# MarkJhonBao/InfantPoseEstimation_GaussianBias

Hardware: AMD Instinct MI355X
Metric: images/sec (train fwd+bwd) HRFormer-S 256x192 (higher is better)
Workload: dtype bf16; 1 GPU; HRFormer-small + fusion head, 256x192 -> 64x48, K=17, train step fwd+bwd+AdamW, DropPath 0.1, BN train; global_batch=64, per_gpu_batch=64, parallelism=dp1, launch=hipGraph replay, branches on concurrent HIP streams

## Files before the change

infantposeestimation_gaussianbias_amd/csrc/pk_layout.hip:

```cpp
#include "pk_rowops.h"

__global__ void __launch_bounds__(256) k_nchw_to_nhwc(const float* __restrict__ x, uint16_t* __restrict__ y, int B, int Cin, int H, int W,
                                                      int Cp, const float* __restrict__ sp_y) {
    const size_t pixels = (size_t)B * H * W;
    for (size_t i = (size_t)blockIdx.x * blockDim.x + threadIdx.x; i < pixels; i += (size_t)gridDim.x * blockDim.x) {
        const size_t b = i / ((size_t)H * W), r = i - b * H * W;
        for (int c0 = 0; c0 < Cp; c0 += 8) {
            float v[8];
#pragma unroll
            for (int j = 0; j < 8; ++j) {
                float t = 0.f;
                if (c0 + j < Cin) {
                    const size_t k = (b * Cin + c0 + j) * H * W + r;
                    t = x[k];
                    if (sp_y) t *= 1.f - __expf(-sp_y[k]);
                }
                v[j] = t;
            }
            *reinterpret_cast<uint4*>(y + i * Cp + c0) = pack8(v);
        }
    }
}
extern "C" int pk_nchw_f32_to_nhwc_bf16(const float* x, const float* softplus_out, void* y, int B, int Cin, int H, int W, int Cpad,
                                        void* stream) {
    PK_REQUIRE(x && y && B > 0 && Cin > 0 && H > 0 && W > 0 && Cpad >= Cin && (Cpad & 7) == 0, "pk_nchw_f32_to_nhwc_bf16: bad argument");
    const size_t pixels = (size_t)B * H * W;
    unsigned gb;
    chunk_grid(pixels, 1, CHUNK_GRID_CAP, nullptr, gb);
    hipLaunchKernelGGL(k_nchw_to_nhwc, dim3(gb), dim3(256), 0, (hipStream_t)stream, x, (uint16_t*)y, B, Cin, H, W, Cpad, softplus_out);
    return pk_launch_status("pk_nchw_f32_to_nhwc_bf16");
}

struct PackDesc { const float* src; int64_t dst_off; int N, C, T, mode, Cp, Np; int64_t dst_numel; };
__global__ void __launch_bounds__(256) k_pack_weights(uint16_t* __restrict__ dst, const PackDesc* __restrict__ desc,
                                                      const int* __restrict__ blk_desc, const int* __restrict__ blk_first) {
    const PackDesc d = desc[blk_desc[blockIdx.x]];
    const float* __restrict__ src = d.src;
    const int64_t i0 = (int64_t)(blockIdx.x - blk_first[blockIdx.x]) * 1024;
    for (int k = 0; k < 4; ++k) {
        const int64_t i = i0 + k * 256 + threadIdx.x;
        if (i >= d.dst_numel) return;
        float v = 0.f;
        if (d.mode == 0) {
            const int c = (int)(i % d.Cp), t = (int)((i / d.Cp) % d.T), n = (int)(i / ((int64_t)d.Cp * d.T));
            if (c < d.C) v = src[((int64_t)n * d.C + c) * d.T + t];
        } else if (d.mode == 1) {
            const int n = (int)(i % d.Np), t = (int)((i / d.Np) % d.T), c = (int)(i / ((int64_t)d.Np * d.T));
            if (n < d.N) v = src[((int64_t)n * d.C + c) * d.T + (d.T - 1 - t)];
        } else {
            const int n = (int)(i % d.Np), c = (int)(i / d.Np);
            if (n < d.N) v = src[(int64_t)n * d.C + c];
        }
        dst[d.dst_off + i] = f32_to_bf16(v);
    }
}
extern "C" int pk_pack_weights(void* flat_dst_bf16, const void* desc_table, const int32_t* block_desc, const int32_t* block_first,
                               int n_blocks, void* stream) {
    PK_REQUIRE(flat_dst_bf16 && desc_table && block_desc && block_first && n_blocks > 0, "pk_pack_weights: bad argument");
    hipLaunchKernelGGL(k_pack_weights, dim3(n_blocks), dim3(256), 0, (hipStream_t)stream, (uint16_t*)flat_dst_bf16,
                       (const PackDesc*)desc_table, block_desc, block_first);
    return pk_launch_status("pk_pack_weights");
}

struct EmbedDesc { float* real; int64_t twin_off; int r[4]; int p[4]; int64_t numel; };
__global__ void __launch_bounds__(256) k_embed_boxes(float* __restrict__ twin, const EmbedDesc* __restrict__ desc,
                                                     const int* __restrict__ blk_desc, const int* __restrict__ blk_first, int direction) {
    const EmbedDesc d = desc[blk_desc[blockIdx.x]];
    const int64_t i0 = (int64_t)(blockIdx.x - blk_first[blockIdx.x]) * 1024;
    for (int k = 0; k < 4; ++k) {
        const int64_t i = i0 + k * 256 + threadIdx.x;
        if (i >= d.numel) return;
        int64_t t = i;
        const int i3 = (int)(t % d.r[3]);
        t /= d.r[3];
        const int i2 = (int)(t % d.r[2]);
        t /= d.r[2];
        const int i1 = (int)(t % d.r[1]), i0_ = (int)(t / d.r[1]);
        const int64_t j = d.twin_off + (((int64_t)i0_ * d.p[1] + i1) * d.p[2] + i2) * d.p[3] + i3;
        if (direction == 0) twin[j] = d.real[i];
        else if (direction == 1) d.real[i] = twin[j];
        else d.real[i] += twin[j];
    }
}
extern "C" int pk_embed_boxes(float* twin_base, const void* desc_table, const int* block_desc, const int* block_first, int n_blocks,
                              int direction, void* stream) {
    PK_REQUIRE(twin_base && desc_table && block_desc && block_first && n_blocks > 0 && direction >= 0 && direction <= 2,
               "pk_embed_boxes: bad argument");
    hipLaunchKernelGGL(k_embed_boxes, dim3(n_blocks), dim3(256), 0, (hipStream_t)stream, twin_base, (const EmbedDesc*)desc_table, block_desc,
                       block_first, direction);
    return pk_launch_status("pk_embed_boxes");
}

__global__ void k_rows_by_map(const uint32_t* __restrict__ src, uint32_t* __restrict__ dst, const int* __restrict__ map, long n_rows,
                              int row_dwords, int scatter) {
    const long total = n_rows * row_dwords;
    for (long i = (long)blockIdx.x * blockDim.x + threadIdx.x; i < total; i += (long)gridDim.x * blockDim.x) {
        const long r = i / row_dwords;
        const int c = (int)(i - r * row_dwords), pr = map[r];
        if (scatter) {
            if (pr >= 0) dst[(long)pr * row_dwords + c] = src[i];
        } else {
            dst[i] = pr >= 0 ? src[(long)pr * row_dwords + c] : 0u;
        }
    }
}
extern "C" int pk_rows_by_map(const void* src, void* dst, const int* rowmap, int64_t n_rows, int row_bytes, int scatter, void* stream) {
    PK_REQUIRE(src && dst && rowmap && n_rows > 0 && row_bytes > 0 && row_bytes % 4 == 0, "pk_rows_by_map: bad argument (rows of whole dwords)");
    const long total = n_rows * (row_bytes / 4);
    const int nb = capped_grid((total + 255) / 256, 4096);
    hipLaunchKernelGGL(k_rows_by_map, dim3(nb), dim3(256), 0, (hipStream_t)stream, (const uint32_t*)src, (uint32_t*)dst, rowmap, (long)n_rows,
                       row_bytes / 4, scatter);
    return pk_launch_status("pk_rows_by_map");
}

__global__ void k_drop_path(const float* __restrict__ x, const float* __restrict__ mask, float* __restrict__ out, long total, long per_sample,
                            float keep) {
    for (long i = (long)blockIdx.x * blockDim.x + threadIdx.x; i < total; i += (long)gridDim.x * blockDim.x)
        out[i] = (x[i] / keep) * mask[i / per_sample];
}
extern "C" int pk_drop_path_f32(const float* x, const float* mask, float* out, int64_t batch, int64_t per_sample, float keep_prob, void* stream) {
    PK_REQUIRE(x && mask && out && batch > 0 && per_sample > 0 && keep_prob > 0.f, "pk_drop_path_f32: bad argument");
    const long total = batch * per_sample;
    const int nb = capped_grid((total + 255) / 256, 4096);
    hipLaunchKernelGGL(k_drop_path, dim3(nb), dim3(256), 0, (hipStream_t)stream, x, mask, out, total, (long)per_sample, keep_prob);
    return pk_launch_status("pk_drop_path_f32");
}
```

Before: 4287 images/sec.

## Tile weight packing through LDS transpose and vectorize contiguous pack path

```diff
diff --git a/infantposeestimation_gaussianbias_amd/csrc/pk_layout.hip b/infantposeestimation_gaussianbias_amd/csrc/pk_layout.hip
--- a/infantposeestimation_gaussianbias_amd/csrc/pk_layout.hip
+++ b/infantposeestimation_gaussianbias_amd/csrc/pk_layout.hip
@@ -32,11 +32,70 @@
 }
 
 struct PackDesc { const float* src; int64_t dst_off; int N, C, T, mode, Cp, Np; int64_t dst_numel; };
+constexpr int PACK_TILE = 64;
+constexpr int PACK_MIN = 32;
+
+__device__ __forceinline__ void pack_tiles(uint16_t* __restrict__ dst, const float* __restrict__ src, int nbatch, int R, int Rp, int Q,
+                                           int T, bool flip, int wg, int n_wg, uint32_t (*tile)[PACK_TILE + 1]) {
+    const int TQ = Q < PACK_TILE ? Q : PACK_TILE;
+    const int tiles_q = (Q + TQ - 1) / TQ, tiles_r = (Rp + PACK_TILE - 1) / PACK_TILE;
+    const int n_tiles = nbatch * tiles_r * tiles_q;
+    for (int tl = wg; tl < n_tiles; tl += n_wg) {
+        const int tq = tl % tiles_q, tr = (tl / tiles_q) % tiles_r, b = tl / (tiles_q * tiles_r);
+        const int r0 = tr * PACK_TILE, q0 = tq * TQ;
+        const int nr = min(PACK_TILE, Rp - r0), nq = min(TQ, Q - q0);
+        const float* __restrict__ s = src + (int64_t)b * R * Q;
+        uint16_t* __restrict__ o = dst + (int64_t)b * Q * Rp;
+        for (int e = threadIdx.x; e < nr * TQ; e += 256) {
+            const int r = TQ == PACK_TILE ? e >> 6 : e / TQ, q = e - r * TQ;
+            float v = 0.f;
+            if (q < nq && r0 + r < R) v = s[(int64_t)(r0 + r) * Q + q0 + q];
+            tile[r][q] = f32_to_bf16(v);
+        }
+        __syncthreads();
+        for (int e = threadIdx.x; e < nq * (PACK_TILE / 2); e += 256) {
+            const int p = e & (PACK_TILE / 2 - 1), q = e >> 5;
+            if (2 * p < nr) {
+                const int qq = q0 + q, fq = flip ? qq - qq % T + (T - 1 - qq % T) : qq;
+                *reinterpret_cast<uint32_t*>(o + (int64_t)fq * Rp + r0 + 2 * p) = tile[2 * p][q] | (tile[2 * p + 1][q] << 16);
+            }
+        }
+        __syncthreads();
+    }
+}
+
 __global__ void __launch_bounds__(256) k_pack_weights(uint16_t* __restrict__ dst, const PackDesc* __restrict__ desc,
                                                       const int* __restrict__ blk_desc, const int* __restrict__ blk_first) {
+    __shared__ uint32_t tile[PACK_TILE][PACK_TILE + 1];
     const PackDesc d = desc[blk_desc[blockIdx.x]];
     const float* __restrict__ src = d.src;
-    const int64_t i0 = (int64_t)(blockIdx.x - blk_first[blockIdx.x]) * 1024;
+    const int wg = blockIdx.x - blk_first[blockIdx.x];
+    const int T = d.mode == 2 ? 1 : d.T;
+    const int R = d.mode == 0 ? d.C : d.N, Rp = d.mode == 0 ? d.Cp : d.Np, Q = d.mode == 0 ? T : d.C * T, nbatch = d.mode == 0 ? d.N : 1;
+    const bool whole = (int64_t)nbatch * Q * Rp == d.dst_numel && Rp >= R;
+    const uintptr_t dst_addr = (uintptr_t)(dst + d.dst_off);
+    if (whole && (dst_addr & 3) == 0 && (Rp & 1) == 0 && Rp >= PACK_MIN && Q >= (d.mode == 0 ? 2 : PACK_MIN)) {
+        pack_tiles(dst + d.dst_off, src, nbatch, R, Rp, Q, T, d.mode != 0, wg, (int)((d.dst_numel + 1023) / 1024), tile);
+        return;
+    }
+    const int64_t i0 = (int64_t)wg * 1024;
+    if (whole && d.mode == 0 && T == 1 && (dst_addr & 7) == 0 && (d.Cp & 3) == 0) {
+        const int64_t i = i0 + threadIdx.x * 4;
+        if (i >= d.dst_numel) return;
+        const int c = (int)(i % d.Cp);
+        const float* p = src + (i / d.Cp) * d.C + c;
+        float4 v = make_float4(0.f, 0.f, 0.f, 0.f);
+        if (c + 3 < d.C && (((uintptr_t)p) & 15) == 0) v = *reinterpret_cast<const float4*>(p);
+        else {
+            if (c < d.C) v.x = p[0];
+            if (c + 1 < d.C) v.y = p[1];
+            if (c + 2 < d.C) v.z = p[2];
+            if (c + 3 < d.C) v.w = p[3];
+        }
+        *reinterpret_cast<uint2*>(dst + d.dst_off + i) = make_uint2(f32_to_bf16(v.x) | ((uint32_t)f32_to_bf16(v.y) << 16),
+                                                                    f32_to_bf16(v.z) | ((uint32_t)f32_to_bf16(v.w) << 16));
+        return;
+    }
     for (int k = 0; k < 4; ++k) {
         const int64_t i = i0 + k * 256 + threadIdx.x;
         if (i >= d.dst_numel) return;
```

Result: no change. 4268 images/sec (-0.4%).
